# telosnetwork/plonky2_goldibear

Measured on AMD Instinct MI355X. Metric: proofs/s, higher is better.
Workload: dtype u64; 1 GPU; prove(): 2^20-row Goldilocks dummy circuit (2^19+1 NoopGates), standard_recursion_config_gl with num_challenges=3, Poseidon-12, witness in page-locked host memory, handed over every step -> proof bytes (198432 B); field=goldilocks, log_n=20, cap_height=4, proofs_in_flight_per_gpu=1, witness=in page-locked host memory, handed over every step

## Files before the change

### plonky2_goldibear_amd/csrc/poseidon_gl_coop.hpp

```cpp
#pragma once
#include "poseidon_gl.hpp"

namespace poseidon_gl_coop {

using gl::u32;
using gl::u64;
using poseidon_gl::FP_VS;
using poseidon_gl::mul_add_lazy;
using poseidon_gl::mul_lazy;
using poseidon_gl::sbox;

__device__ static const u64 WHATS[22 * 11] = {GL_POSEIDON_FAST_PARTIAL_ROUND_W_HATS_LIST};
__device__ static const u64 INIT[11 * 11] = {GL_POSEIDON_FAST_PARTIAL_ROUND_INITIAL_MATRIX_LIST};

__device__ __forceinline__ u64 add_lazy(u64 a, u64 b) {
    u64 s, t;
    const bool c1 = __builtin_uaddll_overflow(a, b, &s);
    const bool c2 = __builtin_uaddll_overflow(s, c1 ? gl::EPS : 0, &t);
    return t + (c2 ? gl::EPS : 0);
}

template <int N>
__device__ __forceinline__ u64 row_ror(u64 x) {
    const int lo = __builtin_amdgcn_update_dpp(0, (int)(u32)x, 0x120 + N, 0xF, 0xF, false);
    const int hi = __builtin_amdgcn_update_dpp(0, (int)(u32)(x >> 32), 0x120 + N, 0xF, 0xF, false);
    return (u64)(u32)lo | ((u64)(u32)hi << 32);
}
__device__ __forceinline__ u64 row_sum(u64 x) {
    x = add_lazy(x, row_ror<8>(x));
    x = add_lazy(x, row_ror<4>(x));
    x = add_lazy(x, row_ror<2>(x));
    return add_lazy(x, row_ror<1>(x));
}

__device__ __forceinline__ u64 permute(u64 x, u32 l, u64* __restrict__ sh) {
    const bool live = l < 12;
    const u32 lc = live ? l : 0;
    x = poseidon_gl::to_mont(x);
    auto mds = [&](u64 v) {
        __syncthreads();
        sh[l] = v;
        __syncthreads();
        u64 sl = 0, shh = 0;
#pragma unroll
        for (int i = 0; i < 12; i++) {
            u32 j = lc + i;
            j = j >= 12 ? j - 12 : j;
            const u64 w = sh[j];
            sl += (u64)(u32)w * poseidon_gl::mds_circ(i);
            shh += (u64)(u32)(w >> 32) * poseidon_gl::mds_circ(i);
        }
        if (l == 0) {
            sl += (u64)(u32)v * poseidon_gl::MDS_DIAG0;
            shh += (u64)(u32)(v >> 32) * poseidon_gl::MDS_DIAG0;
        }
        const u64 t = sl + (shh >> 32) * gl::EPS;
        u64 r;
        const bool cy = __builtin_uaddll_overflow(t, shh << 32, &r);
        r += cy ? gl::EPS : 0;
        return live ? r : 0;
    };
#pragma unroll 1
    for (int r = 0; r < 4; r++) {
        x = add_lazy(x, live ? GB_RC[12 * r + lc] : 0);
        x = mds(sbox(x));
    }
    x = add_lazy(x, live ? GB_FP_FIRST[lc] : 0);
    __syncthreads();
    sh[l] = x;
    __syncthreads();
    u64 s0 = sh[0];
    const bool upper = live && l >= 1;
    const u32 t = upper ? l - 1 : 0;
    {
        u64 acc = 0;
#pragma unroll 1
        for (int r = 1; r < 12; r++) acc = mul_add_lazy(sh[r], INIT[(r - 1) * 11 + t], acc);
        x = upper ? acc : 0;
    }
    const u64 c00 = poseidon_gl::mds_circ(0) + poseidon_gl::MDS_DIAG0;
    u64 wh = upper ? WHATS[t] : c00, vs = FP_VS[t];
#pragma unroll 1
    for (int k = 0; k < 22; k++) {
        const u64 wh_k = wh, vs_k = vs;
        if (k + 1 < 22) {
            wh = upper ? WHATS[11 * (k + 1) + t] : c00;
            vs = FP_VS[11 * (k + 1) + t];
        }
        s0 = add_lazy(sbox(s0), GB_FP_RC[k]);
        const u64 term = mul_lazy(upper ? x : s0, wh_k);
        const u64 upd = mul_add_lazy(s0, vs_k, x);
        x = upper ? upd : 0;
        s0 = row_sum(live ? term : 0);
    }
    if (l == 0) x = s0;
#pragma unroll 1
    for (int r = 0; r < 4; r++) {
        x = add_lazy(x, live ? GB_RC[12 * (4 + 22 + r) + lc] : 0);
        x = mds(sbox(x));
    }
    return poseidon_gl::mont_fold((u32)x, (u32)(x >> 32), 0u, 0u);
}

}
```

Before: 10.89 proofs/s.

## Replace fast partial-round path with plain rounds using fused sbox and RC-in-MDS

Drops the precomputed fast partial-round matrices (INIT, WHATS, VS) and runs all 30 Poseidon rounds as ordinary rounds through the shared-memory MDS, applying the sbox only to lane 0 in partial rounds. A new sbox_coop computes x^3 and x^4 with interleaved Montgomery reductions to raise ILP, and the next round constant is folded into the MDS accumulator instead of a separate add. This removes the DPP row-sum chain and the constant-table loads, but each of the 22 partial rounds now costs two __syncthreads plus a 12-term MDS instead of a row reduction.

New measurement: 11.01 proofs/s (median of 6 runs). +1.1%, better.

```diff
diff --git a/plonky2_goldibear_amd/csrc/poseidon_gl_coop.hpp b/plonky2_goldibear_amd/csrc/poseidon_gl_coop.hpp
--- a/plonky2_goldibear_amd/csrc/poseidon_gl_coop.hpp
+++ b/plonky2_goldibear_amd/csrc/poseidon_gl_coop.hpp
@@ -5,13 +5,6 @@
 
 using gl::u32;
 using gl::u64;
-using poseidon_gl::FP_VS;
-using poseidon_gl::mul_add_lazy;
-using poseidon_gl::mul_lazy;
-using poseidon_gl::sbox;
-
-__device__ static const u64 WHATS[22 * 11] = {GL_POSEIDON_FAST_PARTIAL_ROUND_W_HATS_LIST};
-__device__ static const u64 INIT[11 * 11] = {GL_POSEIDON_FAST_PARTIAL_ROUND_INITIAL_MATRIX_LIST};
 
 __device__ __forceinline__ u64 add_lazy(u64 a, u64 b) {
     u64 s, t;
@@ -19,7 +12,6 @@
     const bool c2 = __builtin_uaddll_overflow(s, c1 ? gl::EPS : 0, &t);
     return t + (c2 ? gl::EPS : 0);
 }
-
 template <int N>
 __device__ __forceinline__ u64 row_ror(u64 x) {
     const int lo = __builtin_amdgcn_update_dpp(0, (int)(u32)x, 0x120 + N, 0xF, 0xF, false);
@@ -33,15 +25,49 @@
     return add_lazy(x, row_ror<1>(x));
 }
 
+__device__ __forceinline__ u64 sbox_coop(u64 x) {
+    const u64 x2 = gl::mul_mont_lazy(x, x);
+    const u32 x0 = (u32)x, x1 = (u32)(x >> 32), y0 = (u32)x2, y1 = (u32)(x2 >> 32);
+    const u64 a00 = (u64)x0 * y0;
+    const u64 b00 = (u64)y0 * y0;
+    const u64 a01 = (u64)x0 * y1 + (a00 >> 32);
+    const u64 b01 = (u64)y0 * y1 + (b00 >> 32);
+    u64 ca, cb;
+    const u64 am = gl::mad_carry(x1, y0, a01, ca);
+    const u64 bm = gl::mad_carry(y1, y0, b01, cb);
+    const u64 a11 = (u64)x1 * y1 + (am >> 32);
+    const u64 b11 = (u64)y1 * y1 + (bm >> 32);
+    const u32 a3 = gl::addc_carry((u32)(a11 >> 32), ca);
+    const u32 b3 = gl::addc_carry((u32)(b11 >> 32), cb);
+    u32 ea, eb, wa, wb, ka, kb;
+    u64 c0a, c0b, cca, ccb, coa, cob;
+    const u32 aa1 = __builtin_addc((u32)am, (u32)a00, 0u, &ea);
+    const u32 ba1 = __builtin_addc((u32)bm, (u32)b00, 0u, &eb);
+    const u32 ab0 = __builtin_subc((u32)a00, aa1, ea, &wa);
+    const u32 bb0 = __builtin_subc((u32)b00, ba1, eb, &wb);
+    const u32 ab1 = __builtin_subc(aa1, 0u, wa, &ka);
+    const u32 bb1 = __builtin_subc(ba1, 0u, wb, &kb);
+    const u32 ar0 = gl::sub_flag((u32)a11, ab0, c0a);
+    const u32 br0 = gl::sub_flag((u32)b11, bb0, c0b);
+    const u32 ar1 = gl::subb_flag(a3, ab1, c0a, cca);
+    const u32 br1 = gl::subb_flag(b3, bb1, c0b, ccb);
+    const u32 af0 = gl::addc_flag(ar0, cca, coa);
+    const u32 bf0 = gl::addc_flag(br0, ccb, cob);
+    const u32 af1 = gl::subb_zero(ar1, cca & ~coa);
+    const u32 bf1 = gl::subb_zero(br1, ccb & ~cob);
+    const u64 x3 = (u64)af0 | ((u64)af1 << 32), x4 = (u64)bf0 | ((u64)bf1 << 32);
+    return gl::mul_mont_lazy(x3, x4);
+}
+
 __device__ __forceinline__ u64 permute(u64 x, u32 l, u64* __restrict__ sh) {
     const bool live = l < 12;
     const u32 lc = live ? l : 0;
     x = poseidon_gl::to_mont(x);
-    auto mds = [&](u64 v) {
+    auto mds = [&](u64 v, u64 c) {
         __syncthreads();
         sh[l] = v;
         __syncthreads();
-        u64 sl = 0, shh = 0;
+        u64 sl = (u32)c, shh = c >> 32;
 #pragma unroll
         for (int i = 0; i < 12; i++) {
             u32 j = lc + i;
@@ -60,44 +86,13 @@
         r += cy ? gl::EPS : 0;
         return live ? r : 0;
     };
+    x = poseidon_gl::add_rc(x, GB_RC[lc]);
 #pragma unroll 1
-    for (int r = 0; r < 4; r++) {
-        x = add_lazy(x, live ? GB_RC[12 * r + lc] : 0);
-        x = mds(sbox(x));
-    }
-    x = add_lazy(x, live ? GB_FP_FIRST[lc] : 0);
-    __syncthreads();
-    sh[l] = x;
-    __syncthreads();
-    u64 s0 = sh[0];
-    const bool upper = live && l >= 1;
-    const u32 t = upper ? l - 1 : 0;
-    {
-        u64 acc = 0;
-#pragma unroll 1
-        for (int r = 1; r < 12; r++) acc = mul_add_lazy(sh[r], INIT[(r - 1) * 11 + t], acc);
-        x = upper ? acc : 0;
-    }
-    const u64 c00 = poseidon_gl::mds_circ(0) + poseidon_gl::MDS_DIAG0;
-    u64 wh = upper ? WHATS[t] : c00, vs = FP_VS[t];
-#pragma unroll 1
-    for (int k = 0; k < 22; k++) {
-        const u64 wh_k = wh, vs_k = vs;
-        if (k + 1 < 22) {
-            wh = upper ? WHATS[11 * (k + 1) + t] : c00;
-            vs = FP_VS[11 * (k + 1) + t];
-        }
-        s0 = add_lazy(sbox(s0), GB_FP_RC[k]);
-        const u64 term = mul_lazy(upper ? x : s0, wh_k);
-        const u64 upd = mul_add_lazy(s0, vs_k, x);
-        x = upper ? upd : 0;
-        s0 = row_sum(live ? term : 0);
-    }
-    if (l == 0) x = s0;
-#pragma unroll 1
-    for (int r = 0; r < 4; r++) {
-        x = add_lazy(x, live ? GB_RC[12 * (4 + 22 + r) + lc] : 0);
-        x = mds(sbox(x));
+    for (int r = 0; r < 30; r++) {
+        const u64 rc = r + 1 < 30 ? GB_RC[12 * (r + 1) + lc] : 0;
+        const u64 y = sbox_coop(x);
+        const bool full = r < 4 || r >= 26;
+        x = mds((full || l == 0) ? y : x, rc);
     }
     return poseidon_gl::mont_fold((u32)x, (u32)(x >> 32), 0u, 0u);
 }
```
